# degleris1/CMF.jl

Hardware: NVIDIA B200
Metric: CNMF iterations/sec (higher is better)
Workload: dtype f32

## Files before the change

cmf.jl_b200/csrc/cmf_sm100.cu:

```cuda
#include "../../include/cmf_sm100.h"

#include <cuda_runtime.h>

#include <algorithm>
#include <chrono>
#include <cmath>
#include <cstdio>
#include <cstring>
#include <map>
#include <memory>
#include <mutex>
#include <tuple>
#include <stdexcept>
#include <string>
#include <vector>

#include <type_traits>

#include "kernels_simt.cuh"
#include "kernels_tc.cuh"
#include "kernels_fd.cuh"
#include "kernels_hals.cuh"
#include "comm.h"

// ... 351 lines not shown
            CK(cudaMemGetInfo(&free_b, &total_b));
            size_t later = (size_t)1 << 30;
            if (alg == CMF_HALS) later += (size_t)2 * (size_t)(Tl + 2048) * (size_t)K * 4 + (size_t)hals2::RING * (size_t)cdiv(K, hals2::GS) * (size_t)K * hals2::CW * 4;
            size_t xf = 0, ah = 0, aw = 0, of = 0, df = 0, hf = 0, gf = 0, ac = 0;
            bool fits = false;
            for (int B = forced ? forced : B0; B <= (forced ? forced : std::min(2 * B0, 1024)); B *= 2) {
                int logB = 0;
                while ((1 << logB) < B) ++logB;
                f.B = B; f.logB = logB; f.V = B - (int)L + 1; f.F = B / 2 + 1;
                f.nblk = cdiv(Tl, f.V);
                f.nblkp = cdiv(f.nblk, 16) * 16;
                xf = (size_t)f.F * (size_t)f.nblkp * 2 * (size_t)N + 64;
                ah = (size_t)f.F * (size_t)f.nblkp * 2 * f.MR + 64;
                aw = (size_t)f.F * f.MR * 2 * (size_t)N + 64;
                f.V2 = B - 2 * (int)L + 2;
                f.nblk2 = cdiv(Tl, f.V2);
                of = (size_t)f.F * (size_t)std::max(f.nblkp, f.nblk2) * f.MR; df = (size_t)f.F * f.MR * (size_t)N;
                hf = (size_t)f.F * (size_t)std::max(f.nblkp, f.nblk2) * 2 * f.Kq + 256; gf = (size_t)f.F * f.MR * f.Kq;
                ac = (size_t)f.F * f.MR * f.MR;
                const size_t need = 4 * (xf + ah + aw + hf + ac) + 4 * (of + df + gf);
                const size_t loss_pass = 4 * aw + (size_t)256 * (size_t)f.F * 2 * (size_t)N * sizeof(float);
                if (need + later + loss_pass <= free_b) { fits = true; break; }
            }
            if (!fits) { f.why = "not enough device memory for the spectrum of X"; return; }
            f.Xf_hi.alloc(xf); f.Xf_lo.alloc(xf);
            f.Ah_hi.alloc(ah); f.Ah_lo.alloc(ah);
            f.Aw_hi.alloc(aw); f.Aw_lo.alloc(aw);
            f.Of.alloc(of); f.Df.alloc(df);
            f.Hf_hi.alloc(hf); f.Hf_lo.alloc(hf); f.Gf.alloc(gf);
            f.Ac_hi.alloc(ac); f.Ac_lo.alloc(ac);
            __nv_bfloat16 *xs[2] = {f.Xf_hi.p, f.Xf_lo.p}, *as[2] = {f.Ah_hi.p, f.Ah_lo.p}, *ws[2] = {f.Aw_hi.p, f.Aw_lo.p};
            const uint64_t rows = (uint64_t)f.F * (uint64_t)f.nblkp;
            for (int i = 0; i < 2; ++i) {
                f.mXfK[i] = make_map_2d(xs[i], (uint64_t)(2 * N), rows, (uint64_t)N * 4, tc::BK, tc::BN, CU_TENSOR_MAP_SWIZZLE_64B);
                f.mXfMN[i] = make_map_mn(xs[i], rows * 2, (uint64_t)N * 2, (uint64_t)cdiv(N, 64), tc::BK, 4);
                f.mAw[i] = make_map_2d(ws[i], (uint64_t)(2 * N), (uint64_t)f.F * f.MR, (uint64_t)N * 4, tc::BK, tc::BM, CU_TENSOR_MAP_SWIZZLE_64B);
                f.mAh[i] = make_map_mn(as[i], rows * 2, (uint64_t)f.MR * 2, (uint64_t)(f.MR / 64), tc::BK, 2);
                f.mHfMN[i] = make_map_mn(i == 0 ? f.Hf_hi.p : f.Hf_lo.p, rows * 2, (uint64_t)f.Kq * 2, (uint64_t)(f.Kq / 64), tc::BK, 4);
                f.mAc[i] = make_map_2d(i == 0 ? f.Ac_hi.p : f.Ac_lo.p, f.MR, (uint64_t)f.F * f.MR, (uint64_t)f.MR * 2, tc::BK, tc::BM, CU_TENSOR_MAP_SWIZZLE_64B);
                f.mHf2K[i] = make_map_2d(i == 0 ? f.Hf_hi.p : f.Hf_lo.p, f.MR, (uint64_t)f.F * (uint64_t)f.nblk2, (uint64_t)f.MR * 2, tc::BK, tc::BN, CU_TENSOR_MAP_SWIZZLE_64B);
            }
            CK(cudaFuncSetAttribute(tc::tc_kernel<tc::TC_FQT>, cudaFuncAttributeMaxDynamicSharedMemorySize, tc::SMEM_BYTES));
            CK(cudaFuncSetAttribute(tc::tc_kernel<tc::TC_FQC>, cudaFuncAttributeMaxDynamicSharedMemorySize, tc::SMEM_BYTES));
            CK(cudaFuncSetAttribute(tc::tc_kernel<tc::TC_FQX>, cudaFuncAttributeMaxDynamicSharedMemorySize, tc::SMEM_BYTES));

            const int big = (int)fd_smem(fd_cols_h()), small_ = (int)fd_smem(16);
            CK(cudaFuncSetAttribute(fd::fft_x_kernel, cudaFuncAttributeMaxDynamicSharedMemorySize, small_));
            CK(cudaFuncSetAttribute(fd::ifft_resid_kernel, cudaFuncAttributeMaxDynamicSharedMemorySize, small_));
            CK(cudaFuncSetAttribute(fd::fft_w_kernel, cudaFuncAttributeMaxDynamicSharedMemorySize, small_));
            CK(cudaFuncSetAttribute(fd::ifft_numW_kernel<float>, cudaFuncAttributeMaxDynamicSharedMemorySize, small_));
            CK(cudaFuncSetAttribute(fd::ifft_numW_kernel<double>, cudaFuncAttributeMaxDynamicSharedMemorySize, small_));
            CK(cudaFuncSetAttribute(fd::fft_h_kernel, cudaFuncAttributeMaxDynamicSharedMemorySize, big));
            CK(cudaFuncSetAttribute(fd::ifft_numH_kernel, cudaFuncAttributeMaxDynamicSharedMemorySize, big));
            f.x_dirty = f.w_dirty = f.h_dirty = true;
            f.ok = true;
        }
    }
    int fd_cols_h() const {
        if (const char *e = getenv("CMF_FD_COLS")) {
            const int c = atoi(e);
            if ((c == 8 || c == 16 || c == 32) && (size_t)fds.B * (size_t)c * sizeof(float2) <= 160 * 1024) return c;
        }
        return fds.B >= 1024 ? 8 : 16;
    }
    int64_t fd_order(int64_t nblocks) const { static const int o = getenv("CMF_FD_ORDER") ? atoi(getenv("CMF_FD_ORDER")) : 0; return o ? nblocks : 0; }
    int fd_cols_w() const { return fds.B >= 1024 ? 8 : 16; }
    size_t fd_smem(int C) const { return ((size_t)fds.B * (size_t)C + (size_t)fds.B) * sizeof(float2); }

    void fd_build_X() {
        if constexpr (std::is_same<S, float>::value) {
            FdState &f = fds;
            if (!f.x_dirty) return;
            dim3 grid((unsigned)(f.nblkp * cdiv(N, 32)));
            fd::fft_x_kernel<<<grid, fd::NT, fd_smem(16), stream>>>(X.p, f.Xf_hi.p, f.Xf_lo.p, N, Tl + (L - 1), f.B, f.logB, f.V, f.nblkp, fd_order(f.nblkp));
            post_launch();
            f.x_dirty = false;
        }
    }
    void fd_corr() {
        if constexpr (std::is_same<S, float>::value) {
            FdState &f = fds;
            fd_build_X();
            fd_spectrum_H();
            tc::Params q = tc_base_params();
            q.nprod = 3;
            q.tiles_n = cdiv(N, tc::BN);
            q.nkb = f.nblkp * 2 / tc::BK;
            q.MR = f.MR; q.mtiles = f.MR / tc::BM; q.units = (int64_t)f.F * q.tiles_n * q.mtiles;
            q.fq_rows = f.nblkp * 2;
            q.out = f.Df.p; q.Mrows = f.MR; q.Ncols = N; q.ldo = N;
            const unsigned grid = (unsigned)std::min<int64_t>(q.units, tcs.num_sms);
            prof_begin(PROF_CORR);
            tc::tc_kernel<tc::TC_FQC><<<grid, tc::THREADS, tc::SMEM_BYTES, stream>>>(f.mAh[0], f.mAh[1], f.mXfMN[0], f.mXfMN[1], q);
            prof_end();
            post_launch();
            fd::ifft_numW_kernel<float><<<dim3((unsigned)cdiv(N, 2 * fd_cols_w()), (unsigned)K), fd::NT, fd_smem(fd_cols_w()), stream>>>(f.Df.p, numW.p, N, N, K, L, f.B, f.logB, f.Kq, fd_cols_w());
            post_launch();
        }
    }
    void fd_denomH() {
        if constexpr (std::is_same<S, float>::value) {
            FdState &f = fds;
            fd::fft_w_kernel<<<dim3((unsigned)cdiv(K, 2 * fd_cols_w()), (unsigned)K), fd::NT, fd_smem(fd_cols_w()), stream>>>(
                Cf.p, f.Ac_hi.p, f.Ac_lo.p, K, K, 2 * L - 1, f.B, f.logB, f.MR, f.Kq, 0, f.Kq, fd_cols_w());
            post_launch();
            const int C = fd_cols_h();
// ... 70 lines not shown
                q.nkb = f.MR / tc::BK;
                q.MR = f.MR; q.mtiles = 1; q.units = (int64_t)f.F * 2 * q.tiles_m * q.tiles_n;
                q.fq_rows = f.nblk; q.b_off = b0; q.nbc = cur;
                q.out = f.Yf.p;
                const unsigned grid = (unsigned)std::min<int64_t>(q.units, tcs.num_sms);
                tc::tc_kernel<tc::TC_FQX><<<grid, tc::THREADS, tc::SMEM_BYTES, stream>>>(f.mAwm[0], f.mAwm[1], f.mHcK[0], f.mHcK[1], q);
                post_launch();
                fd::ifft_resid_kernel<<<(unsigned)(cur * ntile32), fd::NT, fd_smem(16), stream>>>(
                    f.Yf.p, X.p, loss_part.p + b0 * ntile32, N, Tl, L, f.B, f.logB, f.V, cur, b0, fd_order(cur));
                post_launch();
            }
            prof_end();
            return f.nblk * ntile32;
        }
        return 0;
    }
    void fd_spectrum_H() {
        if constexpr (std::is_same<S, float>::value) {
            FdState &f = fds;
            if (!f.h_dirty) return;
            const int C = fd_cols_h();
            fd::fft_h_kernel<<<(unsigned)(f.nblkp * (f.Kq / 2 / C)), fd::NT, fd_smem(C), stream>>>(
                H, f.Ah_hi.p, f.Ah_lo.p, K, Tl, Tl + (L - 1), f.B, f.logB, f.V, f.nblkp, C, 0, 0, f.Kq, fd_order(f.nblkp));
            post_launch();
            f.h_dirty = false;
        }
    }
    void fd_gram() {
        if constexpr (std::is_same<S, float>::value) {
            FdState &f = fds;
            f.hf2_valid = false;
            fd_spectrum_H();
            const int C = fd_cols_h();
            fd::fft_h_kernel<<<(unsigned)(f.nblkp * (f.Kq / 2 / C)), fd::NT, fd_smem(C), stream>>>(
                H, f.Hf_hi.p, f.Hf_lo.p, K, Tl, Tl + (L - 1), f.B, f.logB, f.V, f.nblkp, C, 1, 0, f.Kq, fd_order(f.nblkp));
            post_launch();
            tc::Params q = tc_base_params();
            q.nprod = 3;
            q.tiles_n = 1;
            q.nkb = f.nblkp * 2 / tc::BK;
            q.MR = f.MR; q.mtiles = f.MR / tc::BM; q.units = (int64_t)f.F * q.mtiles;
            q.fq_rows = f.nblkp * 2;
            q.out = f.Gf.p; q.Mrows = f.MR; q.Ncols = K; q.ldo = f.Kq;
            const unsigned grid = (unsigned)std::min<int64_t>(q.units, tcs.num_sms);
            tc::tc_kernel<tc::TC_FQC><<<grid, tc::THREADS, tc::SMEM_BYTES, stream>>>(f.mAh[0], f.mAh[1], f.mHfMN[0], f.mHfMN[1], q);
            post_launch();
            fd::ifft_numW_kernel<double><<<dim3((unsigned)cdiv(K, 2 * fd_cols_w()), (unsigned)K), fd::NT, fd_smem(fd_cols_w()), stream>>>(f.Gf.p, exch1.p, K, f.Kq, K, L, f.B, f.logB, f.Kq, fd_cols_w());
            post_launch();
        }
    }
    void fd_transconv() {
        if constexpr (std::is_same<S, float>::value) {
            FdState &f = fds;
            fd_build_X();
            if (f.w_dirty) {
                fd::fft_w_kernel<<<dim3((unsigned)cdiv(N, 2 * fd_cols_w()), (unsigned)K), fd::NT, fd_smem(fd_cols_w()), stream>>>(Wi.p, f.Aw_hi.p, f.Aw_lo.p, N, K, L, f.B, f.logB, 2 * N, N, 0, f.Kq, fd_cols_w());
                post_launch();
                f.w_dirty = false;
            }
            tc::Params q = tc_base_params();
            q.nprod = 3;
            q.tiles_n = cdiv(f.nblkp, tc::BN);
            q.nkb = cdiv(2 * N, tc::BK);
            q.MR = f.MR; q.mtiles = f.MR / tc::BM; q.units = (int64_t)f.F * q.tiles_n * q.mtiles;
            q.fq_rows = f.nblkp;
            q.out = f.Of.p;
            const unsigned grid = (unsigned)std::min<int64_t>(q.units, tcs.num_sms);
            prof_begin(PROF_TRANSCONV);
            tc::tc_kernel<tc::TC_FQT><<<grid, tc::THREADS, tc::SMEM_BYTES, stream>>>(f.mAw[0], f.mAw[1], f.mXfK[0], f.mXfK[1], q);
            prof_end();
            post_launch();
            const int C = fd_cols_h();
            fd::ifft_numH_kernel<<<(unsigned)(f.nblk * (f.Kq / 2 / C)), fd::NT, fd_smem(C), stream>>>(
                f.Of.p, numH.p, K, Tl, f.B, f.logB, f.V, f.nblkp, C, f.Kq, fd_order(f.nblk));
            post_launch();
        }
    }
    bool tc_available() override {
        if (!tcs.ok && !tcs.tried) tc_setup();
        return tcs.ok;
    }

    void tc_setup() {
        if constexpr (!std::is_same<S, float>::value) { return; } else {
            TcState &t = tcs;
            t.tried = true;
            if (K > 128 || N % 8 != 0) return;
            t.Kp = (int)(cdiv(K, 8) * 8);
            t.G = 128 / t.Kp;
            t.KLp = cdiv(L * t.Kp, 64) * 64;
            t.groups = cdiv(L, t.G);
            t.rows_u = cdiv(L * t.Kp + 128, 128) * 128;
            const int64_t hal = L - 1;
            t.hrows = Tl + hal;
            cudaDeviceProp prop;
            CK(cudaGetDeviceProperties(&prop, device));
            if (prop.major != 10) return;
            t.num_sms = prop.multiProcessorCount;
            t.Wc_hi.alloc((size_t)(N * t.KLp)); t.Wc_lo.alloc((size_t)(N * t.KLp));
            t.Wu_hi.alloc((size_t)(t.rows_u * N)); t.Wu_lo.alloc((size_t)(t.rows_u * N));
            t.groups_c = cdiv(2 * L - 1, t.G);
            t.rows_c = cdiv((2 * L - 1) * t.Kp + 128, 128) * 128;
            t.Cc_hi.alloc((size_t)(t.rows_c * t.Kp)); t.Cc_lo.alloc((size_t)(t.rows_c * t.Kp));
            t.Gc_hi.alloc((size_t)(KL() * t.KLp)); t.Gc_lo.alloc((size_t)(KL() * t.KLp));
            if (GS.n < (size_t)(t.rows_u * t.rows_u)) GS.alloc((size_t)(t.rows_u * t.rows_u));
            __nv_bfloat16 *wc[2] = {t.Wc_hi.p, t.Wc_lo.p};
            __nv_bfloat16 *wu[2] = {t.Wu_hi.p, t.Wu_lo.p};
            for (int i = 0; i < 2; ++i) {
                t.mWc[i] = make_map_2d(wc[i], (uint64_t)t.KLp, (uint64_t)N, (uint64_t)t.KLp * 2, tc::BK, tc::BM, CU_TENSOR_MAP_SWIZZLE_64B);
                t.mWu[i] = make_map_2d(wu[i], (uint64_t)N, (uint64_t)t.rows_u, (uint64_t)N * 2, tc::BK, tc::BM, CU_TENSOR_MAP_SWIZZLE_64B);
                __nv_bfloat16 *cc[2] = {t.Cc_hi.p, t.Cc_lo.p};
                t.mCu[i] = make_map_2d(cc[i], (uint64_t)t.Kp, (uint64_t)t.rows_c, (uint64_t)t.Kp * 2, tc::BK, tc::BM, CU_TENSOR_MAP_SWIZZLE_64B);
                __nv_bfloat16 *gc[2] = {t.Gc_hi.p, t.Gc_lo.p};
                t.mWuB[i] = make_map_2d(wu[i], (uint64_t)N, (uint64_t)t.rows_u, (uint64_t)N * 2, tc::BK, tc::BN, CU_TENSOR_MAP_SWIZZLE_64B);
                t.mWcB[i] = make_map_2d(wc[i], (uint64_t)t.KLp, (uint64_t)N, (uint64_t)t.KLp * 2, tc::BK, tc::BN, CU_TENSOR_MAP_SWIZZLE_64B);
                t.mGc[i] = make_map_2d(gc[i], (uint64_t)t.KLp, (uint64_t)KL(), (uint64_t)t.KLp * 2, tc::BK, tc::BM, CU_TENSOR_MAP_SWIZZLE_64B);
            }
            t.tiles_m = cdiv(t.KLp, tc::BM);
            t.tiles_n = cdiv(N, tc::BN);
            const int64_t tau = Tl + hal, base = t.tiles_m * t.tiles_n;
            double best = -1.0;
            for (int ns = 1; ns <= 16; ++ns) {
                const int64_t sl = cdiv(cdiv(tau, ns), tc::BK) * tc::BK;
                if (ns > 1 && sl < tc::FLUSH_T) break;
                const int64_t units = base * cdiv(tau, sl);
                const double eff = (double)units / (double)(cdiv(units, t.num_sms) * t.num_sms);
                if (eff > best + 1e-9) { best = eff; t.nsplit = (int)cdiv(tau, sl); t.split_len = sl; }
// ... 569 lines not shown
        w_denom_rows(0, KL());
        w_update_rows(l1W, l2W, 0, KL());
    }
    void w_denom_rows(int64_t j0, int64_t j1) override {
        if (tc_active()) {
            tc_denomW(j0, j1);
        } else {
            build_G();
            launch_gemm<false>(GS.p + j0 * KL(), Wi.p, denW.p + j0 * N, j1 - j0, N, KL(), KL(), N, N);
        }
    }
    void w_update_rows(double l1W, double l2W, int64_t j0, int64_t j1) override {
        launch_mu(Wi.p + j0 * N, numW.p + j0 * N, denW.p + j0 * N, l1W, l2W, (j1 - j0) * N);
        mark_w_dirty();
        numH_valid = false; numH_dot_valid = false;
    }
    void w_rows_buffers(void **numw, void **w, int64_t *row_elems) override { *numw = numW.p; *w = Wi.p; *row_elems = N; }

    int64_t s2_ks = 0, s2_ld = 0;

    void lag_tables() {
        if (tc_active()) {
            tc_split_W();
            tc_plain(tcs.mWu, tcs.mWuB, GS.p, tcs.rows_u, tcs.rows_u, N, tcs.rows_u, true);
            s2_ks = tcs.Kp; s2_ld = tcs.rows_u;
        } else {
            launch_gemm<true>(Wi.p, Wi.p, GS.p, KL(), KL(), N, N, N, KL());
            s2_ks = K; s2_ld = KL();
        }
        lag_table_kernel<S><<<(unsigned)cdiv((2 * L - 1) * K * K, 256), 256, 0, stream>>>(GS.p, Cf.p, K, L, s2_ks, s2_ld);
        post_launch();
    }

    DevBuf<double> tail_part;
    void launch_denomH_tail() {
        const int nb = (int)cdiv((2 * L - 1) * K, 256);
        const size_t smem = (size_t)8 * (size_t)(L - 1) * sizeof(double);
        if (getenv("CMF_TAIL_DIRECT") || smem > 48 * 1024) {
            dim3 grid((unsigned)(L - 1), (unsigned)K);
            denomH_tail_kernel<S><<<grid, 256, 0, stream>>>(GS.p, H, denH.p, K, L, Tl, -(L - 1), s2_ks, s2_ld);
            post_launch();
            return;
        }
        const size_t need = (size_t)nb * (size_t)(L - 1) * (size_t)K;
        if (tail_part.n < need) tail_part.alloc(need);
        denomH_tail_prefix_kernel<S><<<dim3((unsigned)nb, (unsigned)K), 256, smem, stream>>>(GS.p, H, tail_part.p, K, L, Tl, -(L - 1), s2_ks, s2_ld);
        post_launch();
        denomH_tail_reduce_kernel<S><<<(unsigned)cdiv((L - 1) * K, 256), 256, 0, stream>>>(tail_part.p, denH.p, K, L, Tl, nb);
        post_launch();
    }

    void h_update(double l1H, double l2H) override {
        REQUIRE(have_data && have_factors, "update: data and factors must be set first");
        if (tc_active()) tc_transconv();
        else launch_transconv(Wi.p, X.p, numH.p, N, K, L, N, Tl, Tl + (L - 1));
        lag_tables();
        if (fd_active()) fd_denomH();
        else if (tc_active()) { tc_split_H(false); tc_denomH(); }
        else launch_transconv(Cf.p, Hbuf.p, denH.p, K, K, 2 * L - 1, K, Tl, Tl + 2 * (L - 1));
        if (is_last && L > 1) {
            launch_denomH_tail();
        }
        numH_dot_valid = launch_mu(H, numH.p, denH.p, l1H, l2H, Tl * K, (loss_mode == 1 && alg == CMF_MULT) ? scal.p + 4 : nullptr);
        numH_valid = (alg == CMF_MULT);
        gram_valid = false; fds.h_dirty = true; fds.hf2_valid = false;
    }

    double *scalars() override { return scal.p; }

    int loss_partial_dev() override {
        REQUIRE(have_data && have_factors, "loss: data and factors must be set first");
        if (loss_mode == 1 && tc_active()) {
            if (!numH_valid && fd_active()) { tc_transconv(); lag_tables(); numH_valid = true; numH_dot_valid = false; }
            if (numH_valid) { loss_partial_expansion_dev(); return 2; }
        }
        int64_t nb = conv_nblocks(0, Tl);
        if (fd_active() && !getenv("CMF_FD_LOSS_TC")) nb = fd_conv_loss();
        else if (tc_active()) nb = tc_conv_loss();
        else launch_conv(Wi.p, H, K, L, -(L - 1), Tl + (L - 1), 0, Tl, 4, nullptr, loss_part.p);
        reduce_scalar(loss_part.p, nb, scal.p);
        CK(cudaMemsetAsync(scal.p + 1, 0, sizeof(double), stream));
        return 1;
    }

    double loss_partial() override {
        const int n = loss_partial_dev();
        double bc[2];
        CK(cudaMemcpyAsync(bc, scal.p, 2 * sizeof(double), cudaMemcpyDeviceToHost, stream));
        CK(cudaStreamSynchronize(stream));
        return n == 2 ? data_sumsq_local - 2.0 * bc[0] + bc[1] : bc[0];
    }

    void loss_partial_expansion_dev() {
        gram_partial();
        gram_valid = true;
        if (getenv("CMF_G_DIRECT"))
            s2_dot_G_kernel<S><<<1024, 256, 0, stream>>>(GS.p, s2_ks, s2_ld, exch1.p, exch1.p + L * K * K, K, L, loss_part.p + 1024);
        else
            s2_dot_G_diag_kernel<S><<<1024, 256, 0, stream>>>(GS.p, s2_ks, s2_ld, exch1.p, exch1.p + L * K * K, K, L, loss_part.p + 1024);
        post_launch();
        reduce_scalar(loss_part.p + 1024, 1024, scal.p + 1);
        if (numH_dot_valid) {
            CK(cudaMemcpyAsync(scal.p, scal.p + 4, sizeof(double), cudaMemcpyDeviceToDevice, stream));
            numH_dot_valid = false;
            return;
        }
// ... 1153 lines not shown
```

cmf.jl_b200/csrc/kernels_fd.cuh:

```cuda
#pragma once
#include <cuda_bf16.h>
#include <cuda_runtime.h>
#include <stdint.h>

namespace cmf {
namespace fd {

#ifndef CMF_FD_MINB
#define CMF_FD_MINB 3
#endif
constexpr int LD_U = 8;
constexpr int NT = 512;
constexpr int KQ_MAX = 128;

__device__ __forceinline__ void make_twiddles(float2 *tw, int B) {
    for (int m = threadIdx.x; m < B; m += NT) {
        float s, c;
        sincospif(-2.0f * (float)m / (float)B, &s, &c);
        tw[m] = make_float2(c, s);
    }
}

__device__ __forceinline__ int rev(int x, int logB) { return (int)(__brev((unsigned)x) >> (32 - logB)); }

__device__ __forceinline__ float2 cmul(float2 a, float2 w) { return make_float2(a.x * w.x - a.y * w.y, a.x * w.y + a.y * w.x); }
__device__ __forceinline__ float2 cadd(float2 a, float2 b) { return make_float2(a.x + b.x, a.y + b.y); }
__device__ __forceinline__ float2 csub(float2 a, float2 b) { return make_float2(a.x - b.x, a.y - b.y); }
template <bool INV> __device__ __forceinline__ float2 mul_mi(float2 a) { return INV ? make_float2(-a.y, a.x) : make_float2(a.y, -a.x); }
template <bool INV> __device__ __forceinline__ float2 mul_w8(float2 a) {
    const float r = 0.70710678118654752f;
    return INV ? make_float2((a.x - a.y) * r, (a.x + a.y) * r) : make_float2((a.x + a.y) * r, (a.y - a.x) * r);
}
template <bool INV> __device__ __forceinline__ float2 mul_w83(float2 a) {
    const float r = 0.70710678118654752f;
    return INV ? make_float2((-a.x - a.y) * r, (a.x - a.y) * r) : make_float2((a.y - a.x) * r, (-a.x - a.y) * r);
}

template <bool INV>
__device__ __forceinline__ void fft_passes(float2 *d, const float2 *tw, int B, int logB, int C) {
    const int c = threadIdx.x % C, j0 = threadIdx.x / C, jstep = NT / C;
    int s = 0;
    for (; s + 2 < logB; s += 3) {
        const int lq = logB - s - 3, q = 1 << lq, qC = q * C;
        for (int j = j0; j < (B >> 3); j += jstep) {
            const int pos = j & (q - 1), g = j >> lq;
            float2 *r = d + ((g << (lq + 3)) + pos) * C + c;
            float2 a0 = r[0], a1 = r[qC], a2 = r[2 * qC], a3 = r[3 * qC], a4 = r[4 * qC], a5 = r[5 * qC], a6 = r[6 * qC], a7 = r[7 * qC];
            float2 t;
            t = csub(a0, a4); a0 = cadd(a0, a4); a4 = t;
            t = csub(a1, a5); a1 = cadd(a1, a5); a5 = mul_w8<INV>(t);
            t = csub(a2, a6); a2 = cadd(a2, a6); a6 = mul_mi<INV>(t);
            t = csub(a3, a7); a3 = cadd(a3, a7); a7 = mul_w83<INV>(t);
            t = csub(a0, a2); a0 = cadd(a0, a2); a2 = t;
            t = csub(a1, a3); a1 = cadd(a1, a3); a3 = mul_mi<INV>(t);
            t = csub(a4, a6); a4 = cadd(a4, a6); a6 = t;
            t = csub(a5, a7); a5 = cadd(a5, a7); a7 = mul_mi<INV>(t);
            t = csub(a0, a1); a0 = cadd(a0, a1); a1 = t;
            t = csub(a2, a3); a2 = cadd(a2, a3); a3 = t;
            t = csub(a4, a5); a4 = cadd(a4, a5); a5 = t;
            t = csub(a6, a7); a6 = cadd(a6, a7); a7 = t;
            if (lq > 0) {
                const int e = pos << s;
                float2 w;
#define CMF_TW(m_, a_) w = tw[(m_) * e]; if (INV) w.y = -w.y; a_ = cmul(a_, w);
                CMF_TW(4, a1) CMF_TW(2, a2) CMF_TW(6, a3) CMF_TW(1, a4) CMF_TW(5, a5) CMF_TW(3, a6) CMF_TW(7, a7)
#undef CMF_TW
            }
            r[0] = a0; r[qC] = a1; r[2 * qC] = a2; r[3 * qC] = a3; r[4 * qC] = a4; r[5 * qC] = a5; r[6 * qC] = a6; r[7 * qC] = a7;
        }
        __syncthreads();
    }
    if (logB - s == 2) {
        for (int j = j0; j < (B >> 2); j += jstep) {
            float2 *r = d + (4 * j) * C + c;
            float2 a0 = r[0], a1 = r[C], a2 = r[2 * C], a3 = r[3 * C], t;
            t = csub(a0, a2); a0 = cadd(a0, a2); a2 = t;
            t = csub(a1, a3); a1 = cadd(a1, a3); a3 = mul_mi<INV>(t);
            r[0] = cadd(a0, a1); r[C] = csub(a0, a1); r[2 * C] = cadd(a2, a3); r[3 * C] = csub(a2, a3);
        }
        __syncthreads();
    } else if (logB - s == 1) {
        for (int j = j0; j < (B >> 1); j += jstep) {
            float2 *r0 = d + (2 * j) * C + c, *r1 = r0 + C;
            const float2 a = *r0, b = *r1;
            *r0 = cadd(a, b);
            *r1 = csub(a, b);
        }
        __syncthreads();
    }
}

__device__ __forceinline__ void unpack_pair(const float2 *d, int f, int B, int logB, int C, int p, float &ar, float &ai, float &br,
                                            float &bi) {
    const float2 z = d[rev(f, logB) * C + p], y = d[rev((B - f) & (B - 1), logB) * C + p];
    ar = 0.5f * (z.x + y.x); ai = 0.5f * (z.y - y.y);
    br = 0.5f * (z.y + y.y); bi = -0.5f * (z.x - y.x);
}

__device__ __forceinline__ void pack_pair(float2 *d, int f, int B, int C, int p, float2 re, float2 im) {
    if (f == 0 || f == B / 2) im = make_float2(0.f, 0.f);
    d[f * C + p] = make_float2(re.x - im.y, im.x + re.y);
    if (f > 0 && f < B / 2) d[(B - f) * C + p] = make_float2(re.x + im.y, re.y - im.x);
}

__device__ __forceinline__ void split2(float a, float b, uint32_t &h, uint32_t &l) {
    const __nv_bfloat162 hh = __floats2bfloat162_rn(a, b);
    const float2 hf = __bfloat1622float2(hh);
    const __nv_bfloat162 ll = __floats2bfloat162_rn(a - hf.x, b - hf.y);
    h = *reinterpret_cast<const uint32_t *>(&hh);
    l = *reinterpret_cast<const uint32_t *>(&ll);
}
__device__ __forceinline__ void store_split2(__nv_bfloat16 *hi, __nv_bfloat16 *lo, int64_t idx, float a, float b) {
    uint32_t h, l;
    split2(a, b, h, l);
    *reinterpret_cast<uint32_t *>(hi + idx) = h;
    *reinterpret_cast<uint32_t *>(lo + idx) = l;
}

__global__ void __launch_bounds__(NT, CMF_FD_MINB)
fft_x_kernel(const float *__restrict__ X, __nv_bfloat16 *__restrict__ hi, __nv_bfloat16 *__restrict__ lo, int64_t N, int64_t xcols,
             int B, int logB, int V, int64_t nblkp, int64_t nbx) {
    extern __shared__ float2 fd_smem[];
    constexpr int C = 16;
    float2 *d = fd_smem, *tw = fd_smem + (size_t)B * C;
    const int ny = (int)((N + 31) / 32);
    const int64_t b = nbx ? blockIdx.x % nbx : blockIdx.x / ny;
    const int p = threadIdx.x % C;
    const int64_t n = (int64_t)(nbx ? blockIdx.x / nbx : blockIdx.x % ny) * 32 + 2 * p;
    make_twiddles(tw, B);
    {
        const int i0 = threadIdx.x / C, istep = NT / C;
        const int64_t lim64 = xcols - b * V;
        const int lim = (n < N) ? (int)(lim64 < 0 ? 0 : (lim64 > B ? B : lim64)) : 0;
        const float *src = X + (b * V + i0) * N + n;
        for (int i = i0; i < B; i += LD_U * istep, src += (int64_t)LD_U * istep * N) {
            float2 v[LD_U];
#pragma unroll
            for (int u = 0; u < LD_U; ++u) {
                v[u] = make_float2(0.f, 0.f);
                if (i + u * istep < lim) v[u] = *reinterpret_cast<const float2 *>(src + (int64_t)u * istep * N);
            }
#pragma unroll
            for (int u = 0; u < LD_U; ++u)
                if (i + u * istep < B) d[(i + u * istep) * C + p] = v[u];
        }
    }
    __syncthreads();
    fft_passes<false>(d, tw, B, logB, C);
    if (n >= N) return;
    for (int f = threadIdx.x / C; f <= B / 2; f += NT / C) {
        float ar, ai, br, bi;
        unpack_pair(d, f, B, logB, C, p, ar, ai, br, bi);
        const int64_t r = ((int64_t)f * nblkp + b) * 2;
        store_split2(hi, lo, r * N + n, ar, br);
        store_split2(hi, lo, (r + 1) * N + n, ai, bi);
    }
}

__global__ void __launch_bounds__(NT, CMF_FD_MINB)
fft_h_kernel(const float *__restrict__ H, __nv_bfloat16 *__restrict__ hi, __nv_bfloat16 *__restrict__ lo, int64_t K, int64_t Tl,
             int64_t hcols, int B, int logB, int V, int64_t nblkp, int C, int full, int64_t t_off, int kq, int64_t nbx) {
    const int64_t KQ = kq, MROWS = 2 * kq;
    extern __shared__ float2 fd_smem[];
    float2 *d = fd_smem, *tw = fd_smem + (size_t)B * C;
    const int ny = (kq / 2) / C;
    const int64_t b = nbx ? blockIdx.x % nbx : blockIdx.x / ny;
    const int p = threadIdx.x % C;
    const int k = 2 * ((int)(nbx ? blockIdx.x / nbx : blockIdx.x % ny) * C + p);
    make_twiddles(tw, B);
    {
        const int i0 = threadIdx.x / C, istep = NT / C;
        const int64_t tb = b * V + t_off;
        const int64_t lim64 = full ? (hcols - tb) : ((Tl - tb < V) ? Tl - tb : V);
        const int lim = (int)(lim64 < 0 ? 0 : (lim64 > B ? B : lim64));
        const float *src = H + (tb + i0) * K + k;
        const bool pair = ((K & 1) == 0) && (k + 1 < K);
        for (int i = i0; i < B; i += LD_U * istep, src += (int64_t)LD_U * istep * K) {
            float2 v[LD_U];
#pragma unroll
            for (int u = 0; u < LD_U; ++u) {
                v[u] = make_float2(0.f, 0.f);
                if (i + u * istep < lim) {
                    const float *q = src + (int64_t)u * istep * K;
                    if (pair) v[u] = *reinterpret_cast<const float2 *>(q);
                    else { if (k < K) v[u].x = q[0]; if (k + 1 < K) v[u].y = q[1]; }
                }
            }
#pragma unroll
            for (int u = 0; u < LD_U; ++u)
                if (i + u * istep < B) d[(i + u * istep) * C + p] = v[u];
        }
    }
    __syncthreads();
    fft_passes<false>(d, tw, B, logB, C);
    for (int f = threadIdx.x / C; f <= B / 2; f += NT / C) {
        float ar, ai, br, bi;
        unpack_pair(d, f, B, logB, C, p, ar, ai, br, bi);
        uint32_t hr, lr, hi_, li_;
        split2(ar, br, hr, lr);
        split2(ai, bi, hi_, li_);
        if (full) {
            const int64_t r = (((int64_t)f * nblkp + b) * 2) * KQ + k;
            *reinterpret_cast<uint32_t *>(hi + r) = hr; *reinterpret_cast<uint32_t *>(lo + r) = lr;
            *reinterpret_cast<uint32_t *>(hi + r + KQ) = hi_; *reinterpret_cast<uint32_t *>(lo + r + KQ) = li_;
            continue;
        }
        const int64_t r = (((int64_t)f * nblkp + b) * 2) * MROWS + k;
        const uint32_t sg = 0x80008000u;
        *reinterpret_cast<uint32_t *>(hi + r) = hr; *reinterpret_cast<uint32_t *>(lo + r) = lr;
        *reinterpret_cast<uint32_t *>(hi + r + KQ) = hi_ ^ sg; *reinterpret_cast<uint32_t *>(lo + r + KQ) = li_ ^ sg;
        *reinterpret_cast<uint32_t *>(hi + r + MROWS) = hi_; *reinterpret_cast<uint32_t *>(lo + r + MROWS) = li_;
        *reinterpret_cast<uint32_t *>(hi + r + MROWS + KQ) = hr; *reinterpret_cast<uint32_t *>(lo + r + MROWS + KQ) = lr;
    }
}

__global__ void __launch_bounds__(NT, CMF_FD_MINB)
fft_w_kernel(const float *__restrict__ Wi, __nv_bfloat16 *__restrict__ hi, __nv_bfloat16 *__restrict__ lo, int64_t N, int64_t K,
             int64_t L, int B, int logB, int64_t ldw, int64_t coff, int xmode, int kq, int C) {
    const int64_t KQ = kq, MROWS = 2 * kq;
    extern __shared__ float2 fd_smem[];
    float2 *d = fd_smem, *tw = fd_smem + (size_t)B * C;
    const int64_t k = blockIdx.y;
    const int p = threadIdx.x % C;
    const int64_t n = (int64_t)blockIdx.x * (2 * C) + 2 * p;
    make_twiddles(tw, B);
    {
        const int i0 = threadIdx.x / C, istep = NT / C;
        for (int i = i0; i < B; i += LD_U * istep) {
            float2 v[LD_U];
#pragma unroll
            for (int u = 0; u < LD_U; ++u) {
                const int ii = i + u * istep;
                v[u] = make_float2(0.f, 0.f);
                if (ii < L && n < N) {
                    const float *src = Wi + ((int64_t)ii * K + k) * N + n;
                    if ((N & 1) == 0) v[u] = *reinterpret_cast<const float2 *>(src);
                    else { v[u].x = src[0]; if (n + 1 < N) v[u].y = src[1]; }
                }
            }
#pragma unroll
            for (int u = 0; u < LD_U; ++u)
                if (i + u * istep < B) d[(i + u * istep) * C + p] = v[u];
        }
    }
    __syncthreads();
    fft_passes<false>(d, tw, B, logB, C);
    if (n >= N) return;
    for (int f = threadIdx.x / C; f <= B / 2; f += NT / C) {
        float ar, ai, br, bi;
        unpack_pair(d, f, B, logB, C, p, ar, ai, br, bi);
        if (xmode) {
            const int64_t r0 = (((int64_t)f * 2 + 0) * MROWS + k) * N + n, r1 = (((int64_t)f * 2 + 1) * MROWS + k) * N + n;
            store_split2(hi, lo, r0, ar, br);
            store_split2(hi, lo, r0 + KQ * N, -ai, -bi);
            store_split2(hi, lo, r1, ai, bi);
            store_split2(hi, lo, r1 + KQ * N, ar, br);
            continue;
        }
        const int64_t re = ((int64_t)f * MROWS + k) * ldw, im = ((int64_t)f * MROWS + KQ + k) * ldw;
        store_split2(hi, lo, re + n, ar, br);
        store_split2(hi, lo, re + coff + n, ai, bi);
        store_split2(hi, lo, im + n, -ai, -bi);
        store_split2(hi, lo, im + coff + n, ar, br);
    }
}

__global__ void __launch_bounds__(NT, CMF_FD_MINB)
ifft_numH_kernel(const float *__restrict__ Of, float *__restrict__ numH, int64_t K, int64_t Tl, int B, int logB, int V,
                 int64_t nblkp, int C, int kq, int64_t nbx) {
    const int64_t KQ = kq, MROWS = 2 * kq;
    extern __shared__ float2 fd_smem[];
    float2 *d = fd_smem, *tw = fd_smem + (size_t)B * C;
    const int ny = (kq / 2) / C;
    const int64_t b = nbx ? blockIdx.x % nbx : blockIdx.x / ny;
    const int p = threadIdx.x % C;
    const int k = 2 * ((int)(nbx ? blockIdx.x / nbx : blockIdx.x % ny) * C + p);
    make_twiddles(tw, B);
    {
        const int f0 = threadIdx.x / C, fstep = NT / C;
        const float *o = Of + ((int64_t)f0 * nblkp + b) * MROWS + k;
        for (int f = f0; f <= B / 2; f += 4 * fstep, o += (int64_t)4 * fstep * nblkp * MROWS) {
            float2 re[4], im[4];
#pragma unroll
            for (int u = 0; u < 4; ++u)
                if (f + u * fstep <= B / 2) {
                    const float *q = o + (int64_t)u * fstep * nblkp * MROWS;
                    re[u] = *reinterpret_cast<const float2 *>(q); im[u] = *reinterpret_cast<const float2 *>(q + KQ);
                }
#pragma unroll
            for (int u = 0; u < 4; ++u)
                if (f + u * fstep <= B / 2) pack_pair(d, f + u * fstep, B, C, p, re[u], im[u]);
        }
    }
    __syncthreads();
    fft_passes<true>(d, tw, B, logB, C);
    const float sc = 1.0f / (float)B;
    const bool pair = ((K & 1) == 0) && (k + 1 < K);
    for (int i = threadIdx.x / C; i < V; i += NT / C) {
        const int64_t t = b * V + i;
        if (t >= Tl) break;
        const float2 z = d[rev(i, logB) * C + p];
        if (pair) *reinterpret_cast<float2 *>(numH + t * K + k) = make_float2(z.x * sc, z.y * sc);
        else { if (k < K) numH[t * K + k] = z.x * sc; if (k + 1 < K) numH[t * K + k + 1] = z.y * sc; }
    }
}

__global__ void __launch_bounds__(NT, CMF_FD_MINB)
ifft_resid_kernel(const float *__restrict__ Yf, const float *__restrict__ X, double *__restrict__ partial, int64_t N, int64_t Tl,
                  int64_t L, int B, int logB, int V, int64_t nbc, int64_t b0, int64_t nbx) {
    extern __shared__ float2 fd_smem[];
    __shared__ double red[NT / 32];
    constexpr int C = 16;
    float2 *d = fd_smem, *tw = fd_smem + (size_t)B * C;
    const int ny = (int)((N + 31) / 32);
    const int64_t bc = nbx ? blockIdx.x % nbx : blockIdx.x / ny;
    const int by = (int)(nbx ? blockIdx.x / nbx : blockIdx.x % ny);
    const int p = threadIdx.x % C;
    const int64_t n = (int64_t)by * 32 + 2 * p;
    make_twiddles(tw, B);
    {
        const int f0 = threadIdx.x / C, fstep = NT / C;
        const float *y = Yf + (((int64_t)f0 * nbc + bc) * 2) * N + n;
        for (int f = f0; f <= B / 2; f += 4 * fstep, y += (int64_t)4 * fstep * nbc * 2 * N) {
            float2 re[4], im[4];
#pragma unroll
            for (int u = 0; u < 4; ++u) {
                re[u] = make_float2(0.f, 0.f); im[u] = re[u];
                if (f + u * fstep <= B / 2 && n < N) {
                    const float *q = y + (int64_t)u * fstep * nbc * 2 * N;
                    re[u] = *reinterpret_cast<const float2 *>(q); im[u] = *reinterpret_cast<const float2 *>(q + N);
                }
            }
#pragma unroll
            for (int u = 0; u < 4; ++u)
                if (f + u * fstep <= B / 2) pack_pair(d, f + u * fstep, B, C, p, re[u], im[u]);
        }
    }
    __syncthreads();
    fft_passes<true>(d, tw, B, logB, C);
    const float sc = 1.0f / (float)B;
    double accd = 0.0;
    if (n < N) {
        const int istep = NT / C;
        const int64_t tb = (b0 + bc) * V - (L - 1);
        for (int i = (int)(L - 1) + threadIdx.x / C; i < B; i += LD_U * istep) {
            float2 x[LD_U];
#pragma unroll
            for (int u = 0; u < LD_U; ++u) {
                const int ii = i + u * istep;
                x[u] = make_float2(0.f, 0.f);
                if (ii < B && tb + ii < Tl) x[u] = *reinterpret_cast<const float2 *>(X + (tb + ii) * N + n);
            }
            float acc = 0.f;
#pragma unroll
            for (int u = 0; u < LD_U; ++u) {
                const int ii = i + u * istep;
                if (ii < B && tb + ii < Tl) {
                    const float2 z = d[rev(ii, logB) * C + p];
                    const float r0 = z.x * sc - x[u].x, r1 = z.y * sc - x[u].y;
                    acc = fmaf(r0, r0, acc);
                    acc = fmaf(r1, r1, acc);
                }
            }
            accd += (double)acc;
        }
    }
#pragma unroll
    for (int o = 16; o > 0; o >>= 1) accd += __shfl_xor_sync(0xffffffffu, accd, o);
    if ((threadIdx.x & 31) == 0) red[threadIdx.x >> 5] = accd;
    __syncthreads();
    if (threadIdx.x == 0) {
        double s = 0.0;
        for (int w = 0; w < NT / 32; ++w) s += red[w];
        partial[bc * ny + by] = s;
    }
}

template <typename OutT>
__global__ void __launch_bounds__(NT, CMF_FD_MINB)
ifft_numW_kernel(const float *__restrict__ Df, OutT *__restrict__ out, int64_t N, int64_t ldi, int64_t K, int64_t L, int B, int logB,
                 int kq, int C) {
    const int64_t KQ = kq, MROWS = 2 * kq;
    extern __shared__ float2 fd_smem[];
    float2 *d = fd_smem, *tw = fd_smem + (size_t)B * C;
    const int64_t k = blockIdx.y;
    const int p = threadIdx.x % C;
    const int64_t n = (int64_t)blockIdx.x * (2 * C) + 2 * p;
    make_twiddles(tw, B);
    {
        const int f0 = threadIdx.x / C, fstep = NT / C;
        for (int f = f0; f <= B / 2; f += 4 * fstep) {
            float2 re[4], im[4];
#pragma unroll
            for (int u = 0; u < 4; ++u) {
                const int ff = f + u * fstep;
                re[u] = make_float2(0.f, 0.f); im[u] = re[u];
                if (ff <= B / 2 && n < N) {
                    re[u] = *reinterpret_cast<const float2 *>(Df + ((int64_t)ff * MROWS + k) * ldi + n);
                    im[u] = *reinterpret_cast<const float2 *>(Df + ((int64_t)ff * MROWS + KQ + k) * ldi + n);
                }
            }
#pragma unroll
            for (int u = 0; u < 4; ++u)
                if (f + u * fstep <= B / 2) pack_pair(d, f + u * fstep, B, C, p, re[u], im[u]);
        }
    }
    __syncthreads();
    fft_passes<true>(d, tw, B, logB, C);
    if (n >= N) return;
    const float sc = 1.0f / (float)B;
    for (int l = threadIdx.x / C; l < L; l += NT / C) {
        const float2 z = d[rev(l, logB) * C + p];
        OutT *o = out + ((int64_t)l * K + k) * N + n;
        if (sizeof(OutT) == 4) {
            *reinterpret_cast<float2 *>(o) = make_float2(z.x * sc, z.y * sc);
        } else {
            o[0] = (OutT)(z.x * sc);
            if (n + 1 < N) o[1] = (OutT)(z.y * sc);
        }
    }
}

}
}
```

Baseline: 20.80.

## Fuse H multiplicative update with inverse and forward FFT in one kernel

Adds a fused kernel for the multiplicative H update in the frequency-domain path. It takes the inverse FFT of the numerator, applies the MU update to H in place, optionally accumulates the loss dot product, and runs the forward FFT to rebuild the bf16 hi/lo frequency operands for H, all in one launch. This removes separate passes and global round trips for numH, the H update and the fft_h step. It also folds the final radix-2 FFT stage into the unpack and output reads whenever logB mod 3 is 1, which saves one shared-memory pass plus a sync. The cost is more complex code and higher per-block work, and the in-place bit-reversal swap and fold logic could hide correctness bugs.

```diff
diff --git a/cmf.jl_b200/csrc/cmf_sm100.cu b/cmf.jl_b200/csrc/cmf_sm100.cu
--- a/cmf.jl_b200/csrc/cmf_sm100.cu
+++ b/cmf.jl_b200/csrc/cmf_sm100.cu
@@ -427,6 +427,7 @@
             CK(cudaFuncSetAttribute(fd::ifft_numW_kernel<double>, cudaFuncAttributeMaxDynamicSharedMemorySize, small_));
             CK(cudaFuncSetAttribute(fd::fft_h_kernel, cudaFuncAttributeMaxDynamicSharedMemorySize, big));
             CK(cudaFuncSetAttribute(fd::ifft_numH_kernel, cudaFuncAttributeMaxDynamicSharedMemorySize, big));
+            CK(cudaFuncSetAttribute(fd::mu_h_fused_kernel, cudaFuncAttributeMaxDynamicSharedMemorySize, big));
             f.x_dirty = f.w_dirty = f.h_dirty = true;
             f.ok = true;
         }
@@ -603,6 +604,31 @@
     void fd_transconv() {
         if constexpr (std::is_same<S, float>::value) {
             FdState &f = fds;
+            fd_numH_product();
+            const int C = fd_cols_h();
+            fd::ifft_numH_kernel<<<(unsigned)(f.nblk * (f.Kq / 2 / C)), fd::NT, fd_smem(C), stream>>>(
+                f.Of.p, numH.p, K, Tl, f.B, f.logB, f.V, f.nblkp, C, f.Kq, fd_order(f.nblk));
+            post_launch();
+        }
+    }
+    void fd_mu_h(double l1, double l2, double *dot_dst) {
+        if constexpr (std::is_same<S, float>::value) {
+            FdState &f = fds;
+            fd_numH_product();
+            const int C = fd_cols_h();
+            const unsigned grid = (unsigned)(f.nblkp * (f.Kq / 2 / C));
+            if (dot_dst && mu_part.n < grid) mu_part.alloc(grid);
+            fd::mu_h_fused_kernel<<<grid, fd::NT, fd_smem(C), stream>>>(
+                f.Of.p, numH.p, H, denH.p, f.Ah_hi.p, f.Ah_lo.p, dot_dst ? mu_part.p : nullptr, (float)l1, (float)l2, K, Tl, f.B,
+                f.logB, f.V, f.nblkp, C, f.Kq, fd_order(f.nblkp));
+            post_launch();
+            if (dot_dst) reduce_scalar(mu_part.p, grid, dot_dst);
+            f.h_dirty = false;
+        }
+    }
+    void fd_numH_product() {
+        if constexpr (std::is_same<S, float>::value) {
+            FdState &f = fds;
             fd_build_X();
             if (f.w_dirty) {
                 fd::fft_w_kernel<<<dim3((unsigned)cdiv(N, 2 * fd_cols_w()), (unsigned)K), fd::NT, fd_smem(fd_cols_w()), stream>>>(Wi.p, f.Aw_hi.p, f.Aw_lo.p, N, K, L, f.B, f.logB, 2 * N, N, 0, f.Kq, fd_cols_w());
@@ -620,10 +646,6 @@
             prof_begin(PROF_TRANSCONV);
             tc::tc_kernel<tc::TC_FQT><<<grid, tc::THREADS, tc::SMEM_BYTES, stream>>>(f.mAw[0], f.mAw[1], f.mXfK[0], f.mXfK[1], q);
             prof_end();
-            post_launch();
-            const int C = fd_cols_h();
-            fd::ifft_numH_kernel<<<(unsigned)(f.nblk * (f.Kq / 2 / C)), fd::NT, fd_smem(C), stream>>>(
-                f.Of.p, numH.p, K, Tl, f.B, f.logB, f.V, f.nblkp, C, f.Kq, fd_order(f.nblk));
             post_launch();
         }
     }
@@ -1299,6 +1321,16 @@
 
     void h_update(double l1H, double l2H) override {
         REQUIRE(have_data && have_factors, "update: data and factors must be set first");
+        if (fd_active() && alg == CMF_MULT) {
+            lag_tables();
+            fd_denomH();
+            if (is_last && L > 1) launch_denomH_tail();
+            fd_mu_h(l1H, l2H, loss_mode == 1 ? scal.p + 4 : nullptr);
+            numH_dot_valid = (loss_mode == 1);
+            numH_valid = true;
+            gram_valid = false; fds.hf2_valid = false;
+            return;
+        }
         if (tc_active()) tc_transconv();
         else launch_transconv(Wi.p, X.p, numH.p, N, K, L, N, Tl, Tl + (L - 1));
         lag_tables();
diff --git a/cmf.jl_b200/csrc/kernels_fd.cuh b/cmf.jl_b200/csrc/kernels_fd.cuh
--- a/cmf.jl_b200/csrc/kernels_fd.cuh
+++ b/cmf.jl_b200/csrc/kernels_fd.cuh
@@ -36,8 +36,9 @@
     return INV ? make_float2((-a.x - a.y) * r, (a.x - a.y) * r) : make_float2((a.y - a.x) * r, (-a.x - a.y) * r);
 }
 
+__device__ __forceinline__ bool fold_last(int logB) { return logB % 3 == 1; }
 template <bool INV>
-__device__ __forceinline__ void fft_passes(float2 *d, const float2 *tw, int B, int logB, int C) {
+__device__ __forceinline__ void fft_passes(float2 *d, const float2 *tw, int B, int logB, int C, bool fold = false) {
     const int c = threadIdx.x % C, j0 = threadIdx.x / C, jstep = NT / C;
     int s = 0;
     for (; s + 2 < logB; s += 3) {
@@ -79,7 +80,7 @@
             r[0] = cadd(a0, a1); r[C] = csub(a0, a1); r[2 * C] = cadd(a2, a3); r[3 * C] = csub(a2, a3);
         }
         __syncthreads();
-    } else if (logB - s == 1) {
+    } else if (logB - s == 1 && !fold) {
         for (int j = j0; j < (B >> 1); j += jstep) {
             float2 *r0 = d + (2 * j) * C + c, *r1 = r0 + C;
             const float2 a = *r0, b = *r1;
@@ -90,11 +91,31 @@
     }
 }
 
-__device__ __forceinline__ void unpack_pair(const float2 *d, int f, int B, int logB, int C, int p, float &ar, float &ai, float &br,
-                                            float &bi) {
-    const float2 z = d[rev(f, logB) * C + p], y = d[rev((B - f) & (B - 1), logB) * C + p];
-    ar = 0.5f * (z.x + y.x); ai = 0.5f * (z.y - y.y);
-    br = 0.5f * (z.y + y.y); bi = -0.5f * (z.x - y.x);
+__device__ __forceinline__ void row_pair(const float2 *d, int r, int C, int p, bool fold, float2 &z0, float2 &z1) {
+    const float2 a = d[r * C + p], b = d[(r + 1) * C + p];
+    z0 = fold ? cadd(a, b) : a;
+    z1 = fold ? csub(a, b) : b;
+}
+__device__ __forceinline__ float2 row_out(const float2 *d, int r, int C, int p, bool fold) {
+    if (!fold) return d[r * C + p];
+    const float2 a = d[(r & ~1) * C + p], b = d[(r | 1) * C + p];
+    return (r & 1) ? csub(a, b) : cadd(a, b);
+}
+
+template <typename Emit>
+__device__ __forceinline__ void for_each_bin(const float2 *d, int B, int logB, int C, int p, Emit emit) {
+    const bool fold = fold_last(logB);
+    auto unpack = [&](int f, float2 z, float2 y) {
+        emit(f, 0.5f * (z.x + y.x), 0.5f * (z.y - y.y), 0.5f * (z.y + y.y), -0.5f * (z.x - y.x));
+    };
+    for (int f = threadIdx.x / C; f <= B / 4; f += NT / C) {
+        float2 zf, zf2, zg, zg2;
+        row_pair(d, rev(f, logB), C, p, fold, zf, zf2);
+        const int g = (B / 2 - f) & (B / 2 - 1);
+        row_pair(d, rev(g, logB), C, p, fold, zg, zg2);
+        unpack(f, zf, f ? zg2 : zf);
+        if (2 * f != B / 2) unpack(B / 2 - f, f ? zg : zf2, zf2);
+    }
 }
 
 __device__ __forceinline__ void pack_pair(float2 *d, int f, int B, int C, int p, float2 re, float2 im) {
@@ -146,15 +167,22 @@
         }
     }
     __syncthreads();
-    fft_passes<false>(d, tw, B, logB, C);
+    fft_passes<false>(d, tw, B, logB, C, fold_last(logB));
     if (n >= N) return;
-    for (int f = threadIdx.x / C; f <= B / 2; f += NT / C) {
-        float ar, ai, br, bi;
-        unpack_pair(d, f, B, logB, C, p, ar, ai, br, bi);
+    for_each_bin(d, B, logB, C, p, [&](int f, float ar, float ai, float br, float bi) {
         const int64_t r = ((int64_t)f * nblkp + b) * 2;
         store_split2(hi, lo, r * N + n, ar, br);
         store_split2(hi, lo, (r + 1) * N + n, ai, bi);
-    }
+    });
+}
+
+__device__ __forceinline__ void store_ah(__nv_bfloat16 *hi, __nv_bfloat16 *lo, int64_t r, int64_t KQ, int64_t MROWS, uint32_t hr,
+                                         uint32_t lr, uint32_t hi_, uint32_t li_) {
+    const uint32_t sg = 0x80008000u;
+    *reinterpret_cast<uint32_t *>(hi + r) = hr; *reinterpret_cast<uint32_t *>(lo + r) = lr;
+    *reinterpret_cast<uint32_t *>(hi + r + KQ) = hi_ ^ sg; *reinterpret_cast<uint32_t *>(lo + r + KQ) = li_ ^ sg;
+    *reinterpret_cast<uint32_t *>(hi + r + MROWS) = hi_; *reinterpret_cast<uint32_t *>(lo + r + MROWS) = li_;
+    *reinterpret_cast<uint32_t *>(hi + r + MROWS + KQ) = hr; *reinterpret_cast<uint32_t *>(lo + r + MROWS + KQ) = lr;
 }
 
 __global__ void __launch_bounds__(NT, CMF_FD_MINB)
@@ -192,10 +220,8 @@
         }
     }
     __syncthreads();
-    fft_passes<false>(d, tw, B, logB, C);
-    for (int f = threadIdx.x / C; f <= B / 2; f += NT / C) {
-        float ar, ai, br, bi;
-        unpack_pair(d, f, B, logB, C, p, ar, ai, br, bi);
+    fft_passes<false>(d, tw, B, logB, C, fold_last(logB));
+    for_each_bin(d, B, logB, C, p, [&](int f, float ar, float ai, float br, float bi) {
         uint32_t hr, lr, hi_, li_;
         split2(ar, br, hr, lr);
         split2(ai, bi, hi_, li_);
@@ -203,15 +229,10 @@
             const int64_t r = (((int64_t)f * nblkp + b) * 2) * KQ + k;
             *reinterpret_cast<uint32_t *>(hi + r) = hr; *reinterpret_cast<uint32_t *>(lo + r) = lr;
             *reinterpret_cast<uint32_t *>(hi + r + KQ) = hi_; *reinterpret_cast<uint32_t *>(lo + r + KQ) = li_;
-            continue;
-        }
-        const int64_t r = (((int64_t)f * nblkp + b) * 2) * MROWS + k;
-        const uint32_t sg = 0x80008000u;
-        *reinterpret_cast<uint32_t *>(hi + r) = hr; *reinterpret_cast<uint32_t *>(lo + r) = lr;
-        *reinterpret_cast<uint32_t *>(hi + r + KQ) = hi_ ^ sg; *reinterpret_cast<uint32_t *>(lo + r + KQ) = li_ ^ sg;
-        *reinterpret_cast<uint32_t *>(hi + r + MROWS) = hi_; *reinterpret_cast<uint32_t *>(lo + r + MROWS) = li_;
-        *reinterpret_cast<uint32_t *>(hi + r + MROWS + KQ) = hr; *reinterpret_cast<uint32_t *>(lo + r + MROWS + KQ) = lr;
-    }
+        } else {
+            store_ah(hi, lo, (((int64_t)f * nblkp + b) * 2) * MROWS + k, KQ, MROWS, hr, lr, hi_, li_);
+        }
+    });
 }
 
 __global__ void __launch_bounds__(NT, CMF_FD_MINB)
@@ -244,25 +265,23 @@
         }
     }
     __syncthreads();
-    fft_passes<false>(d, tw, B, logB, C);
+    fft_passes<false>(d, tw, B, logB, C, fold_last(logB));
     if (n >= N) return;
-    for (int f = threadIdx.x / C; f <= B / 2; f += NT / C) {
-        float ar, ai, br, bi;
-        unpack_pair(d, f, B, logB, C, p, ar, ai, br, bi);
+    for_each_bin(d, B, logB, C, p, [&](int f, float ar, float ai, float br, float bi) {
         if (xmode) {
             const int64_t r0 = (((int64_t)f * 2 + 0) * MROWS + k) * N + n, r1 = (((int64_t)f * 2 + 1) * MROWS + k) * N + n;
             store_split2(hi, lo, r0, ar, br);
             store_split2(hi, lo, r0 + KQ * N, -ai, -bi);
             store_split2(hi, lo, r1, ai, bi);
             store_split2(hi, lo, r1 + KQ * N, ar, br);
-            continue;
+            return;
         }
         const int64_t re = ((int64_t)f * MROWS + k) * ldw, im = ((int64_t)f * MROWS + KQ + k) * ldw;
         store_split2(hi, lo, re + n, ar, br);
         store_split2(hi, lo, re + coff + n, ai, bi);
         store_split2(hi, lo, im + n, -ai, -bi);
         store_split2(hi, lo, im + coff + n, ar, br);
-    }
+    });
 }
 
 __global__ void __launch_bounds__(NT, CMF_FD_MINB)
@@ -293,16 +312,106 @@
         }
     }
     __syncthreads();
-    fft_passes<true>(d, tw, B, logB, C);
+    const bool fold = fold_last(logB);
+    fft_passes<true>(d, tw, B, logB, C, fold);
     const float sc = 1.0f / (float)B;
     const bool pair = ((K & 1) == 0) && (k + 1 < K);
-    for (int i = threadIdx.x / C; i < V; i += NT / C) {
+    auto put = [&](int i, float2 z) {
         const int64_t t = b * V + i;
-        if (t >= Tl) break;
-        const float2 z = d[rev(i, logB) * C + p];
+        if (i >= V || t >= Tl) return;
         if (pair) *reinterpret_cast<float2 *>(numH + t * K + k) = make_float2(z.x * sc, z.y * sc);
         else { if (k < K) numH[t * K + k] = z.x * sc; if (k + 1 < K) numH[t * K + k + 1] = z.y * sc; }
-    }
+    };
+    for (int i = threadIdx.x / C; i < B / 2 && i < V && b * V + i < Tl; i += NT / C) {
+        float2 z0, z1;
+        row_pair(d, rev(i, logB), C, p, fold, z0, z1);
+        put(i, z0);
+        put(i + B / 2, z1);
+    }
+}
+
+__global__ void __launch_bounds__(NT, CMF_FD_MINB)
+mu_h_fused_kernel(const float *__restrict__ Of, float *__restrict__ numH, float *__restrict__ H, const float *__restrict__ denH,
+                  __nv_bfloat16 *__restrict__ hi, __nv_bfloat16 *__restrict__ lo, double *__restrict__ partial, float l1, float l2,
+                  int64_t K, int64_t Tl, int B, int logB, int V, int64_t nblkp, int C, int kq, int64_t nbx) {
+    const int64_t KQ = kq, MROWS = 2 * kq;
+    extern __shared__ float2 fd_smem[];
+    __shared__ double red[NT / 32];
+    float2 *d = fd_smem, *tw = fd_smem + (size_t)B * C;
+    const int ny = (kq / 2) / C;
+    const int64_t b = nbx ? blockIdx.x % nbx : blockIdx.x / ny;
+    const int p = threadIdx.x % C;
+    const int k = 2 * ((int)(nbx ? blockIdx.x / nbx : blockIdx.x % ny) * C + p);
+    make_twiddles(tw, B);
+    {
+        const int f0 = threadIdx.x / C, fstep = NT / C;
+        const float *o = Of + ((int64_t)f0 * nblkp + b) * MROWS + k;
+        for (int f = f0; f <= B / 2; f += 4 * fstep, o += (int64_t)4 * fstep * nblkp * MROWS) {
+            float2 re[4], im[4];
+#pragma unroll
+            for (int u = 0; u < 4; ++u)
+                if (f + u * fstep <= B / 2) {
+                    const float *q = o + (int64_t)u * fstep * nblkp * MROWS;
+                    re[u] = *reinterpret_cast<const float2 *>(q); im[u] = *reinterpret_cast<const float2 *>(q + KQ);
+                }
+#pragma unroll
+            for (int u = 0; u < 4; ++u)
+                if (f + u * fstep <= B / 2) pack_pair(d, f + u * fstep, B, C, p, re[u], im[u]);
+        }
+    }
+    __syncthreads();
+    fft_passes<true>(d, tw, B, logB, C);
+    const float sc = 1.0f / (float)B, eps = (float)CMF_EPS;
+    const bool pair = ((K & 1) == 0) && (k + 1 < K);
+    double acc = 0.0;
+    auto step = [&](int i, float2 z) -> float2 {
+        const int64_t t = b * V + i;
+        float2 h = make_float2(0.f, 0.f);
+        if (i >= V || t >= Tl || k >= K) return h;
+        const float2 a = make_float2(z.x * sc, z.y * sc);
+        float2 dn = make_float2(0.f, 0.f);
+        float *hp = H + t * K + k;
+        if (pair) {
+            *reinterpret_cast<float2 *>(numH + t * K + k) = a;
+            h = *reinterpret_cast<const float2 *>(hp);
+            dn = *reinterpret_cast<const float2 *>(denH + t * K + k);
+        } else {
+            numH[t * K + k] = a.x; h.x = hp[0]; dn.x = denH[t * K + k];
+            if (k + 1 < K) { numH[t * K + k + 1] = a.y; h.y = hp[1]; dn.y = denH[t * K + k + 1]; }
+        }
+        h.x = h.x * (a.x / (dn.x + l1 + 2.f * l2 * h.x + eps)); h.x = h.x > eps ? h.x : eps;
+        if (pair || k + 1 < K) { h.y = h.y * (a.y / (dn.y + l1 + 2.f * l2 * h.y + eps)); h.y = h.y > eps ? h.y : eps; }
+        if (pair) *reinterpret_cast<float2 *>(hp) = h;
+        else { hp[0] = h.x; if (k + 1 < K) hp[1] = h.y; }
+        acc += (double)a.x * (double)h.x + (double)a.y * (double)h.y;
+        return h;
+    };
+    for (int i = threadIdx.x / C; i < B; i += NT / C) {
+        const int r = rev(i, logB);
+        if (r < i) continue;
+        const float2 zi = d[r * C + p], zr = d[i * C + p];
+        const float2 hi_ = step(i, zi);
+        if (r != i) d[r * C + p] = step(r, zr);
+        d[i * C + p] = hi_;
+    }
+    if (partial) {
+#pragma unroll
+        for (int o = 16; o > 0; o >>= 1) acc += __shfl_xor_sync(0xffffffffu, acc, o);
+        if ((threadIdx.x & 31) == 0) red[threadIdx.x >> 5] = acc;
+    }
+    __syncthreads();
+    if (partial && threadIdx.x == 0) {
+        double s = 0.0;
+        for (int w = 0; w < NT / 32; ++w) s += red[w];
+        partial[blockIdx.x] = s;
+    }
+    fft_passes<false>(d, tw, B, logB, C, fold_last(logB));
+    for_each_bin(d, B, logB, C, p, [&](int f, float ar, float ai, float br, float bi) {
+        uint32_t hr, lr, hi2, li2;
+        split2(ar, br, hr, lr);
+        split2(ai, bi, hi2, li2);
+        store_ah(hi, lo, (((int64_t)f * nblkp + b) * 2) * MROWS + k, KQ, MROWS, hr, lr, hi2, li2);
+    });
 }
 
 __global__ void __launch_bounds__(NT, CMF_FD_MINB)
@@ -337,7 +446,8 @@
         }
     }
     __syncthreads();
-    fft_passes<true>(d, tw, B, logB, C);
+    const bool fold = fold_last(logB);
+    fft_passes<true>(d, tw, B, logB, C, fold);
     const float sc = 1.0f / (float)B;
     double accd = 0.0;
     if (n < N) {
@@ -356,7 +466,7 @@
             for (int u = 0; u < LD_U; ++u) {
                 const int ii = i + u * istep;
                 if (ii < B && tb + ii < Tl) {
-                    const float2 z = d[rev(ii, logB) * C + p];
+                    const float2 z = row_out(d, rev(ii, logB), C, p, fold);
                     const float r0 = z.x * sc - x[u].x, r1 = z.y * sc - x[u].y;
                     acc = fmaf(r0, r0, acc);
                     acc = fmaf(r1, r1, acc);
@@ -406,11 +516,12 @@
         }
     }
     __syncthreads();
-    fft_passes<true>(d, tw, B, logB, C);
+    const bool fold = fold_last(logB);
+    fft_passes<true>(d, tw, B, logB, C, fold);
     if (n >= N) return;
     const float sc = 1.0f / (float)B;
     for (int l = threadIdx.x / C; l < L; l += NT / C) {
-        const float2 z = d[rev(l, logB) * C + p];
+        const float2 z = row_out(d, rev(l, logB), C, p, fold);
         OutT *o = out + ((int64_t)l * K + k) * N + n;
         if (sizeof(OutT) == 4) {
             *reinterpret_cast<float2 *>(o) = make_float2(z.x * sc, z.y * sc);
```

New measurement: 21.85, median of 6. +5.0%, better.
